# yezhen17/3DIoUMatch

Measured on AMD Instinct MI355X. Metric: scenes/sec train-step (ScanNet 40k pts, 256 proposals), higher is better.
Workload: dtype f32

## Files before the change

3dioumatch_amd/csrc/mlp_bwd_fused.hip:

```cpp
#include "common.h"
#include "mlp_operand.h"
#include "mlp_bwd_x6.h"

#ifndef MLP_LIN4_OCC
#define MLP_LIN4_OCC 1
#endif

namespace {

template <int MB, int KB, int KBD, int NB, int PMODE, int QMODE, int OCC, bool STATS, bool DGRAD = true,
          bool X6 = false>
__global__ void __launch_bounds__(256, OCC)
gemm_bwd_fused_kernel(int k_total, int r, int total_chunks, int chunks_per_cloud, int xyz,
                      OperandB opp, OperandB opq, const float *__restrict__ w,
                      float *__restrict__ dq, float *__restrict__ part,
                      float *__restrict__ stats_part) {
  constexpr int M = 32 * MB, KP = 32 * KB, TN = 32 * NB;
  constexpr int LDP = M + 1, LDQ = KP + 1;
  constexpr int TPR = TN / 16;
  constexpr int RPP = 256 / TPR;
  constexpr int PP = (M + RPP - 1) / RPP, QP = (KP + RPP - 1) / RPP;
  constexpr int WMB = MB >= 4 ? MB / 4 : 1;
  constexpr int WKB = MB >= 4 ? KB : KB * MB / 4;
  static_assert(MB >= 4 ? MB % 4 == 0 : (MB == 2 && KB % 2 == 0), "dW blocks must split over 4 waves");
// ... 285 lines not shown
#pragma unroll
            for (int n = 0; n < DN; ++n)
              accD[e][n] = __builtin_amdgcn_mfma_f32_32x32x2f32(wreg[e][g * DU + u], bp[g & 1][u][n],
                                                                accD[e][n], 0, 0, 0);
        between(g);
        __builtin_amdgcn_sched_barrier(0);
      }
      }
#pragma unroll
      for (int e = 0; e < (TF ? 0 : DK); ++e) {
        const int kbd = KBD >= 4 ? wave * DK + e : (wave >> 1);
#pragma unroll
        for (int n = 0; n < DN; ++n) {
          const int nb = KBD >= 4 ? n : (wave & 1);
          float *dst = dq + ((size_t)b * k_total + xyz + 32 * kbd + 4 * lhi) * r + col0 + nb * 32 + l31;
#pragma unroll
          for (int q = 0; q < 16; ++q)
            __builtin_nontemporal_store(accD[e][n][q], &dst[(size_t)((q & 3) + 8 * (q >> 2)) * r]);
        }
      }
    }

    auto stats_row = [&](int q) {
      const int ro = (q & 3) + 8 * (q >> 2);
      if constexpr (TF) {
#pragma unroll
        for (int e = 0; e < DK; ++e) {
          const int kbd = KBD >= 4 ? wave * DK + e : (wave >> 1);
#pragma unroll
          for (int n = 0; n < DN; ++n) {
            const int nb = KBD >= 4 ? n : (wave & 1);
            const int col = nb * 32 + 4 * lhi + ro;
            const float yv = Qc[col * LDQ + 32 * kbd + l31];
            const float g = __fmaf_rn(yv, trc[e].x, trc[e].y) > 0.f ? accD[e][n][q] : 0.f;
            st1[e][0] += g;
            st2[e][0] = __fmaf_rn(g, (yv - trc[e].z) * trc[e].w, st2[e][0]);
            const float4 xc = X4s[cur][col];
            gx[e][0] = __fmaf_rn(g, xc.x, gx[e][0]);
            gx[e][1] = __fmaf_rn(g, xc.y, gx[e][1]);
            gx[e][2] = __fmaf_rn(g, xc.z, gx[e][2]);
            gx[e][3] = __fmaf_rn(g, xc.w, gx[e][3]);
          }
        }
        return;
      }
#pragma unroll
      for (int e = 0; e < DK; ++e) {
        const int kbd = KBD >= 4 ? wave * DK + e : (wave >> 1);
        const float4 rc = Rc[32 * kbd + 4 * lhi + ro];
#pragma unroll
        for (int n = 0; n < DN; ++n) {
          const int nb = KBD >= 4 ? n : (wave & 1);
          const float yv = Qc[(nb * 32 + l31) * LDQ + 32 * kbd + 4 * lhi + ro];
          const float g = __fmaf_rn(yv, rc.x, rc.y) > 0.f ? accD[e][n][q] : 0.f;
          st1[e][STATS ? q : 0] += g;
          st2[e][STATS ? q : 0] = __fmaf_rn(g, (yv - rc.z) * rc.w, st2[e][STATS ? q : 0]);
        }
      }
    };
    if constexpr (X6) {
      float qraw[8];
      auto qfrag = [&](int g, int j) {
        const int kb = MB >= 4 ? j : (wave / MB) + (4 / MB) * j;
#pragma unroll
        for (int jj = 0; jj < 8; ++jj) {
          const float raw = Qc[(16 * g + 8 * lhi + jj) * LDQ + kb * 32 + l31];
          qraw[jj] = RAWQ ? fmaxf(__fmaf_rn(raw, fsc[j], fsh[j]), 0.f) : raw;
        }
      };
#pragma unroll
      for (int g = 0; g < WG; ++g) {
        Split3 sp[WMB];
#pragma unroll
        for (int i = 0; i < WMB; ++i) {
          const int mb = MB >= 4 ? wave + 4 * i : wave % MB;
          float praw[8];
#pragma unroll
          for (int jj = 0; jj < 8; ++jj) praw[jj] = Pc[(16 * g + 8 * lhi + jj) * LDP + mb * 32 + l31];
          sp[i] = split3(praw);
        }
        qfrag(g, 0);
#pragma unroll
        for (int j = 0; j < WKB; ++j) {
          const Split3 sq = split3(qraw);
          if (j + 1 < WKB) qfrag(g, j + 1);
#pragma unroll
          for (int i = 0; i < WMB; ++i) mfma_x6(accW[i][j], sp[i], sq);
        }
        between(DG + g);
        if (STATS) {
#pragma unroll
          for (int q = g * 16 / WG; q < (g + 1) * 16 / WG; ++q) stats_row(q);
        }
      }
    } else {
      float ap[2][WU][WMB], bq[2][WU][WKB];
      auto frag = [&](int g, float (&a)[WU][WMB], float (&bb)[WU][WKB]) {
#pragma unroll
        for (int u = 0; u < WU; ++u) {
          const int n = 2 * (g * WU + u) + lhi;
#pragma unroll
          for (int i = 0; i < WMB; ++i) {
            const int mb = MB >= 4 ? wave + 4 * i : wave % MB;
            a[u][i] = Pc[n * LDP + mb * 32 + l31];
          }
#pragma unroll
          for (int j = 0; j < WKB; ++j) {
            const int kb = MB >= 4 ? j : (wave / MB) + (4 / MB) * j;
            const float raw = Qc[n * LDQ + kb * 32 + l31];
            bb[u][j] = RAWQ ? fmaxf(__fmaf_rn(raw, fsc[j], fsh[j]), 0.f) : raw;
          }
        }
      };
      frag(0, ap[0], bq[0]);
#pragma unroll
      for (int g = 0; g < WG; ++g) {
        if (g + 1 < WG) frag(g + 1, ap[(g + 1) & 1], bq[(g + 1) & 1]);
        __builtin_amdgcn_sched_barrier(0);
#pragma unroll
        for (int u = 0; u < WU; ++u)
#pragma unroll
          for (int i = 0; i < WMB; ++i)
#pragma unroll
            for (int j = 0; j < WKB; ++j)
              accW[i][j] = __builtin_amdgcn_mfma_f32_32x32x2f32(ap[g & 1][u][i], bq[g & 1][u][j],
                                                                accW[i][j], 0, 0, 0);
        between(DG + g);
        if (STATS) {
#pragma unroll
          for (int q = g * 16 / WG; q < (g + 1) * 16 / WG; ++q) stats_row(q);
        }
        __builtin_amdgcn_sched_barrier(0);
      }
    }

    if (DGRAD && NB == 1 && xyz) {
      const int n = tid & 31, g8 = tid >> 5;
      float s0 = 0.f, s1 = 0.f, s2 = 0.f;
#pragma unroll 4
      for (int mm = g8 * (M / 8); mm < (g8 + 1) * (M / 8); ++mm) {
        const float pv = Pc[n * LDP + mm];
        s0 = __fmaf_rn(pv, Wx[mm], s0);
        s1 = __fmaf_rn(pv, Wx[M + mm], s1);
        s2 = __fmaf_rn(pv, Wx[2 * M + mm], s2);
      }
      red[(g8 * 3 + 0) * 32 + n] = s0;
      red[(g8 * 3 + 1) * 32 + n] = s1;
      red[(g8 * 3 + 2) * 32 + n] = s2;
      __syncthreads();
      if (tid < 96) {
        const int kx = tid >> 5;
        float t = 0.f;
#pragma unroll
        for (int g = 0; g < 8; ++g) t += red[(g * 3 + kx) * 32 + n];
        dq[((size_t)b * k_total + kx) * r + col0 + n] = t;
      }
    }
    __syncthreads();
  }

  if constexpr (TF) {
    constexpr int PPW = KBD >= 4 ? 1 : 2;
    const int parts = (int)gridDim.x * PPW;
    const int pidx = (int)blockIdx.x * PPW + (KBD >= 4 ? 0 : (wave & 1));
#pragma unroll
    for (int e = 0; e < DK; ++e) {
      const int row = 32 * (KBD >= 4 ? wave * DK + e : (wave >> 1)) + l31;
      float a1 = st1[e][0], a2 = st2[e][0];
      a1 += __shfl_xor(a1, 32, kWave);
      a2 += __shfl_xor(a2, 32, kWave);
      float g4[4];
#pragma unroll
      for (int k = 0; k < 4; ++k) g4[k] = gx[e][k] + __shfl_xor(gx[e][k], 32, kWave);
      if (lhi == 0) {
        if (stats_part != nullptr) {
          stats_part[((size_t)row * parts + pidx) * 2] = a1;
          stats_part[((size_t)row * parts + pidx) * 2 + 1] = a2;
        }
        *reinterpret_cast<float4 *>(dq + ((size_t)pidx * k_total + row) * 4) = make_float4(g4[0], g4[1], g4[2], g4[3]);
      }
    }
  } else if (STATS && stats_part != nullptr) {
    constexpr int PPW = KBD >= 4 ? 1 : 2;
    const int parts = (int)gridDim.x * PPW;
    const int pidx = (int)blockIdx.x * PPW + (KBD >= 4 ? 0 : (wave & 1));
#pragma unroll
    for (int e = 0; e < DK; ++e) {
      const int kbd = KBD >= 4 ? wave * DK + e : (wave >> 1);
#pragma unroll
      for (int q = 0; q < SQ; ++q) {
        float a1 = st1[e][q], a2 = st2[e][q];
#pragma unroll
        for (int off = 1; off < 32; off <<= 1) {
          a1 += __shfl_xor(a1, off, kWave);
          a2 += __shfl_xor(a2, off, kWave);
        }
        if (l31 == 0) {
          const int row = 32 * kbd + 4 * lhi + (q & 3) + 8 * (q >> 2);
          stats_part[((size_t)row * parts + pidx) * 2] = a1;
          stats_part[((size_t)row * parts + pidx) * 2 + 1] = a2;
        }
      }
    }
  }
  float *out = part + (size_t)blockIdx.x * M * k_total;
#pragma unroll
  for (int i = 0; i < WMB; ++i) {
    const int mb = MB >= 4 ? wave + 4 * i : wave % MB;
#pragma unroll
    for (int j = 0; j < WKB; ++j) {
      const int kb = MB >= 4 ? j : (wave / MB) + (4 / MB) * j;
      const int colk = kb * 32 + l31;
      if (colk >= k_total) continue;
#pragma unroll
      for (int q = 0; q < 16; ++q) {
        const int row = mb * 32 + (q & 3) + 8 * (q >> 2) + 4 * lhi;
        out[(size_t)row * k_total + colk] = accW[i][j][q];
      }
    }
  }
}

struct FusedShape { int m, k, xyz, tn, occ; };

bool fused_shape(int m, int k, FusedShape *s) {
  static const FusedShape table[] = {
      {64, 64, 0, 64, 2}, {128, 64, 0, 64, 1}, {128, 128, 0, 32, 2},
      {256, 128, 0, 32, 1}, {128, 131, 3, 32, 1}, {128, 259, 3, 32, 1},
  };
  for (const FusedShape &t : table)
    if (t.m == m && t.k == k) { *s = t; return true; }
  return false;
}

int fused_workgroups(const FusedShape &s, long long total_chunks) {
  long long g = (long long)pn2_cu_count() * s.occ;
  if (g > total_chunks / 8) g = total_chunks / 8;
  return (int)(g < 1 ? 1 : g);
}

}

#define MLP_API extern "C" __attribute__((visibility("default")))

MLP_API int mlp_gemm_backward_fused_supported(int b, int m, int k, int r, int pmode, int qmode,
                                              int ns) {
  FusedShape s;
  if (b <= 0 || r <= 0 || !fused_shape(m, k, &s)) return 0;
  if (r % s.tn != 0 || (long long)b * (r / s.tn) < 64) return 0;
  if (pmode != OP_DY && pmode != OP_POOLDY) return 0;
  if (pmode == OP_POOLDY && (ns <= 0 || ns % 16 != 0 || r % ns != 0 || (ns % s.tn != 0 && s.tn % ns != 0)))
    return 0;
  if (qmode == OP_LIN4) return m == 64 && k == 64 && pmode == OP_DY;
  const bool first = s.xyz != 0;
  if (first != (qmode == OP_DIRECT)) return 0;
  if (qmode != OP_DIRECT && qmode != OP_BNRELU) return 0;
  const bool pooled_only = (m == 128 && k == 64) || (m == 256 && k == 128);
  const bool either = m == 128 && k == 128;
  if (!either && pooled_only != (pmode == OP_POOLDY)) return 0;
  return 1;
}

MLP_API int mlp_gemm_backward_fused_stats_parts(int b, int m, int k, int r) {
  FusedShape s;
  const int gx = mlp_bwd_x6_workgroups(b, m, k, r, pn2_cu_count());
  if (gx > 0) return gx;
  if (!fused_shape(m, k, &s) || k != 64 || r % s.tn != 0) return 0;
  return fused_workgroups(s, (long long)b * (r / s.tn)) * 2;
}

MLP_API size_t mlp_gemm_backward_fused_workspace_floats(int b, int m, int k, int r) {
  FusedShape s;
  if (!fused_shape(m, k, &s) || r % s.tn != 0) return 0;
  const long long g0 = fused_workgroups(s, (long long)b * (r / s.tn));
  const long long g1 = mlp_bwd_x6_workgroups(b, m, k, r, pn2_cu_count());
  return (size_t)(g0 > g1 ? g0 : g1) * m * k;
}

MLP_API int mlp_gemm_backward_fused(int b, int m, int k, int r, const float *w, const MlpOperand *dy,
                                    const MlpOperand *x, float *dq, float *dw, float *workspace,
                                    float *stats_part, void *stream_) {
  if (b <= 0 || m <= 0 || k <= 0 || r <= 0) return 0;
  OperandB P, Q;
  int orc = operand_from_abi(dy, op_bit(OP_DY) | op_bit(OP_POOLDY), r, &P);
  if (!orc) orc = operand_from_abi(x, op_bit(OP_DIRECT) | op_bit(OP_BNRELU) | op_bit(OP_LIN4), r, &Q);
  if (orc) return orc;
  const int pmode = dy->mode, qmode = x->mode;
  if (qmode != OP_DIRECT && (!Q.mean || !Q.invstd)) return (int)hipErrorInvalidValue;
  if (!mlp_gemm_backward_fused_supported(b, m, k, r, pmode, qmode, P.ns)) return (int)hipErrorInvalidValue;
  FusedShape s;
  fused_shape(m, k, &s);
  if (dq == nullptr && !(m == 128 && k == 259)) return (int)hipErrorInvalidValue;
  hipStream_t stream = (hipStream_t)stream_;
  const int cpc = r / s.tn;
  const int total = b * cpc;
  const int g = fused_workgroups(s, total);
  {
    int gx = 0;
    const int rcx = mlp_bwd_x6_try(b, m, k, r, pmode, qmode, P, Q, w, dq, workspace,
                                   qmode == OP_BNRELU ? stats_part : nullptr, pn2_cu_count(), &gx, stream);
    if (rcx > 0) return rcx;
    if (rcx == 0) return mlp_reduce_weight_partials(m * k, gx, workspace, dw, stream);
  }
  if (k != 64) stats_part = nullptr;
#define FUSED_X(MB, KB, KBD, NB, PM, QM, OCC, ST, X6)                                           \
  hipLaunchKernelGGL((gemm_bwd_fused_kernel<MB, KB, KBD, NB, PM, QM, OCC, ST, true, X6>), dim3(g), \
                     dim3(256), 0, stream, k, r, total, cpc, s.xyz, P, Q, w, dq, workspace,     \
                     stats_part)
#define FUSED(MB, KB, KBD, NB, PM, QM, OCC, ST) FUSED_X(MB, KB, KBD, NB, PM, QM, OCC, ST, true)
#define FUSED_F32(MB, KB, KBD, NB, PM, QM, OCC, ST) FUSED_X(MB, KB, KBD, NB, PM, QM, OCC, ST, false)
  if (m == 64 && k == 64 && qmode == OP_LIN4) FUSED(2, 2, 2, 2, OP_DY, OP_LIN4, MLP_LIN4_OCC, true);
  else if (m == 64 && k == 64) FUSED(2, 2, 2, 2, OP_DY, OP_BNRELU, 2, true);
  else if (m == 128 && k == 64) FUSED(4, 2, 2, 2, OP_POOLDY, OP_BNRELU, 1, true);
  else if (m == 256 && k == 128) FUSED(8, 4, 4, 1, OP_POOLDY, OP_BNRELU, 1, false);
  else if (m == 128 && k == 131) FUSED(4, 5, 4, 1, OP_DY, OP_DIRECT, 1, false);
  else if (dq != nullptr) FUSED_F32(4, 9, 8, 1, OP_DY, OP_DIRECT, 1, false);
  else
    hipLaunchKernelGGL((gemm_bwd_fused_kernel<4, 9, 8, 1, OP_DY, OP_DIRECT, 1, false, false, true>), dim3(g),
                       dim3(256), 0, stream, k, r, total, cpc, s.xyz, P, Q, w, dq, workspace, stats_part);
#undef FUSED_F32
#undef FUSED
#undef FUSED_X
  int rc = pn2_launch_status();
  if (rc) return rc;
  return mlp_reduce_weight_partials(m * k, g, workspace, dw, stream);
}
```

3dioumatch_amd/csrc/mlp_bwd_x6.h:

```cpp
#pragma once
#include "common.h"
#include "mlp_operand.h"
#include <type_traits>

namespace {

#if defined(BWDX6_ABL) && BWDX6_ABL == 2
#define mfma_x6(ACC, A, B) do { (ACC)[0] += __builtin_bit_cast(float, (int)(A).hi[0] + (int)(B).hi[0] + (int)(A).mid[1] + (int)(B).mid[1] + (int)(A).lo[2] + (int)(B).lo[2]); } while (0)
#endif

#ifndef BWDX6_DGRAD_SLICES_STATS
#define BWDX6_DGRAD_SLICES_STATS 0xC0u
#endif
#ifndef BWDX6_DGRAD_SLICES_PLAIN
#define BWDX6_DGRAD_SLICES_PLAIN 0xF0u
#endif

constexpr int x6_popcount(unsigned v) { return v == 0 ? 0 : (int)(v & 1u) + x6_popcount(v >> 1); }

template <int MB, int KB, int KBD, int PMODE, int QMODE, bool STATS, bool DGRAD>
__device__ __forceinline__ void gemm_bwd_x6_role(int k_total, int r, int total_chunks,
                                                 int chunks_per_cloud, int xyz, const OperandB &P,
                                                 const OperandB &Q, const float *__restrict__ w,
                                                 float *__restrict__ dq, float *__restrict__ part,
// ... 64 lines not shown
      }
    }
  }

  f32x16 accW[WMB][WKB];
  if (!DGRAD) {
#pragma unroll
    for (int i = 0; i < WMB; ++i)
#pragma unroll
      for (int j = 0; j < WKB; ++j)
#pragma unroll
        for (int q = 0; q < 16; ++q) accW[i][j][q] = 0.f;
  }

  const int per = (total_chunks + (int)gridDim.x - 1) / (int)gridDim.x;
  const int c_lo = (int)blockIdx.x * per;
  const int c_hi = c_lo + per < total_chunks ? c_lo + per : total_chunks;

  float4 px[PS], pd[PS], qx[QS];
  int pwin[PS];
  float pdp[PS];
#pragma unroll
  for (int p = 0; p < PS; ++p) {
    pwin[p] = -1; pdp[p] = 0.f;
    px[p] = make_float4(0.f, 0.f, 0.f, 0.f); pd[p] = px[p];
  }
#pragma unroll
  for (int q = 0; q < QS; ++q) qx[q] = make_float4(0.f, 0.f, 0.f, 0.f);

  struct ChunkAt { size_t p, q, grp; int s0; };
  auto chunk_at = [&](int c) {
    const int b = c / chunks_per_cloud;
    const int col0 = (c - b * chunks_per_cloud) * TN;
    ChunkAt at;
    at.p = (size_t)b * M * r + col0;
    at.q = (size_t)b * k_total * r + col0;
    at.grp = 0; at.s0 = 0;
    if (PMODE == OP_POOLDY) {
      const int g0 = col0 / P.ns;
      at.grp = (size_t)b * M * P.groups + g0;
      at.s0 = col0 - g0 * P.ns;
    }
    return at;
  };
  auto fetch_slice = [&](int sl, const ChunkAt &at) {
    if (sl < PS) {
      const int p = sl;
      px[p] = *reinterpret_cast<const float4 *>(P.x + at.p + p_lane[p]);
      if (PMODE == OP_DY) {
        pd[p] = *reinterpret_cast<const float4 *>(P.dz + at.p + p_lane[p]);
      } else if (PMODE == OP_POOLDY) {
        const size_t gi = at.grp + (size_t)(seg_row + p * 32) * P.groups + lane_g;
        pwin[p] = P.argmax[gi] - (at.s0 + lane_s);
        pdp[p] = P.dz[gi];
      }
    } else {
      const int q = sl - PS;
      qx[q] = *reinterpret_cast<const float4 *>(Q.x + at.q + q_lane[q]);
    }
  };
  auto stage_slice = [&](int sl, int buf) {
    char *base = lds + (size_t)buf * BUF;
    if (sl < PS) {
      const int p = sl;
      const float xv[4] = {px[p].x, px[p].y, px[p].z, px[p].w};
      const float dv[4] = {pd[p].x, pd[p].y, pd[p].z, pd[p].w};
      float v[4];
#pragma unroll
      for (int e = 0; e < 4; ++e) {
        const float dz = PMODE == OP_POOLDY ? (e == pwin[p] ? pdp[p] : 0.f) : dv[e];
        v[e] = transform<PMODE>(xv[e], dz, pc[p]);
      }
      store_split4<RP>(base, PIMG, seg_row + p * 32, seg_c, v);
    } else {
      const int q = sl - PS;
      const float xv[4] = {qx[q].x, qx[q].y, qx[q].z, qx[q].w};
      float v[4];
#pragma unroll
      for (int e = 0; e < 4; ++e) v[e] = q_ok[q] ? transform<QMODE>(xv[e], 0.f, qc[q]) : 0.f;
      store_split4<RP>(base + 3 * PIMG, QIMG, seg_row + q * 32, seg_c, v);
      if (STATS)
        *reinterpret_cast<float4 *>(base + 3 * (PIMG + QIMG) + (size_t)(seg_row + q * 32) * RAWP + seg_c * 4) =
            qx[q];
    }
  };

  auto clampc = [&](int c) { return c < c_hi ? c : c_hi - 1; };
  if (NOWN > 0 && c_lo < c_hi) {
    const ChunkAt first = chunk_at(c_lo), second = chunk_at(clampc(c_lo + 1));
#pragma unroll
    for (int sl = 0; sl < NS; ++sl)
      if (X6_MINE(sl)) fetch_slice(sl, first);
#pragma unroll
    for (int sl = 0; sl < NS; ++sl) {
      if (!X6_MINE(sl)) continue;
      stage_slice(sl, 0);
      fetch_slice(sl, second);
    }
  }
  __syncthreads();

  const int tr_off = (8 * lhi + ((lane & 15) >> 2)) * RP + (16 * ((lane >> 4) & 1) + 4 * (lane & 3)) * 2;
  const int rw_off = l31 * RP + 8 * lhi * 2;

  auto chunk = [&](int c, int cur) {
    const char *Pc = lds + (size_t)cur * BUF, *Qc = Pc + 3 * PIMG;
    const ChunkAt ahead = chunk_at(clampc(c + 2));
    auto between = [&](int g) {
#if !defined(BWDX6_ABL) || BWDX6_ABL != 1
      int own = 0;
#pragma unroll
      for (int sl = 0; sl < NS; ++sl) {
        if (!X6_MINE(sl)) continue;
        if (own >= g * NOWN / NG && own < (g + 1) * NOWN / NG) {
#if !defined(BWDX6_ABL) || BWDX6_ABL != 7
          stage_slice(sl, cur ^ 1);
#else
          if (sl < PS) asm volatile("" :: "v"(px[sl].x), "v"(px[sl].w), "v"(pd[sl].x), "v"(pd[sl].w), "v"(pdp[sl]), "v"(pwin[sl]));
          else asm volatile("" :: "v"(qx[sl - PS].x), "v"(qx[sl - PS].w));
#endif
#if !defined(BWDX6_ABL) || BWDX6_ABL != 6
          fetch_slice(sl, ahead);
#endif
        }
        ++own;
      }
#endif
    };

    if (DGRAD) {
      const int b = c / chunks_per_cloud;
      const int col0 = (c - b * chunks_per_cloud) * TN;
      f32x16 accD[DK];
#pragma unroll
      for (int e = 0; e < DK; ++e)
#pragma unroll
        for (int q = 0; q < 16; ++q) accD[e][q] = 0.f;
      bf16x4 pf[2][3][2];
      auto frag = [&](int s, bf16x4 (&dst)[3][2]) {
#pragma unroll
        for (int t = 0; t < 3; ++t) {
          const char *p0 = Pc + (size_t)t * PIMG + (size_t)(16 * s) * RP + tr_off;
          dst[t][0] = lds_read_tr(p0);
          dst[t][1] = lds_read_tr(p0 + 4 * RP);
        }
      };
#if defined(BWDX6_ABL) && BWDX6_ABL == 3
#pragma unroll
      for (int s = 0; s < DG; ++s) between(s);
#else
      frag(0, pf[0]);
#pragma unroll
      for (int s = 0; s < DG; ++s) {
        if (s + 1 < DG) frag(s + 1, pf[(s + 1) & 1]);
        Split3 sb;
        sb.hi = __builtin_shufflevector(pf[s & 1][0][0], pf[s & 1][0][1], 0, 1, 2, 3, 4, 5, 6, 7);
        sb.mid = __builtin_shufflevector(pf[s & 1][1][0], pf[s & 1][1][1], 0, 1, 2, 3, 4, 5, 6, 7);
        sb.lo = __builtin_shufflevector(pf[s & 1][2][0], pf[s & 1][2][1], 0, 1, 2, 3, 4, 5, 6, 7);
#pragma unroll
        for (int e = 0; e < DK; ++e) mfma_x6(accD[e], wsp[e][s], sb);
        between(s);
      }
#endif
#if !defined(BWDX6_ABL) || (BWDX6_ABL != 5 && BWDX6_ABL != 3)
#pragma unroll
      for (int e = 0; e < DK; ++e) {
        const int kbd = wave * DK + e;
        float *dst = dq + ((size_t)b * k_total + xyz + 32 * kbd + 4 * lhi) * r + col0 + l31;
#pragma unroll
        for (int q = 0; q < 16; ++q) {
#if defined(BWDX6_PLAIN_STORES)
          dst[(size_t)((q & 3) + 8 * (q >> 2)) * r] = accD[e][q];
#else
          __builtin_nontemporal_store(accD[e][q], &dst[(size_t)((q & 3) + 8 * (q >> 2)) * r]);
#endif
        }
      }
#endif
      if (STATS) {
        const float4 *rc = reinterpret_cast<const float4 *>(lds + RCOFF);
        const char *raw = Pc + 3 * (PIMG + QIMG);
#pragma unroll
        for (int q = 0; q < 16; ++q) {
          const int ro = (q & 3) + 8 * (q >> 2);
#pragma unroll
          for (int e = 0; e < DK; ++e) {
            const int row = 32 * (wave * DK + e) + 4 * lhi + ro;
            const float4 c4 = rc[row];
            const float yv = *reinterpret_cast<const float *>(raw + (size_t)row * RAWP + l31 * 4);
            const float g = __fmaf_rn(yv, c4.x, c4.y) > 0.f ? accD[e][q] : 0.f;
            st1[e][q] += g;
            st2[e][q] = __fmaf_rn(g, (yv - c4.z) * c4.w, st2[e][q]);
          }
        }
      }
    } else {
      Split3 sp[WMB], sq[2];
      auto pfrag = [&](int s) {
#pragma unroll
        for (int i = 0; i < WMB; ++i) {
          const char *p0 = Pc + (size_t)((wave + 4 * i) * 32) * RP + rw_off + 16 * s * 2;
          sp[i].hi = *reinterpret_cast<const bf16x8 *>(p0);
          sp[i].mid = *reinterpret_cast<const bf16x8 *>(p0 + PIMG);
          sp[i].lo = *reinterpret_cast<const bf16x8 *>(p0 + 2 * PIMG);
        }
      };
      auto qfrag = [&](int u, Split3 &dst) {
        const int s = u / WKB, j = u % WKB;
        const char *q0 = Qc + (size_t)(j * 32) * RP + rw_off + 16 * s * 2;
        dst.hi = *reinterpret_cast<const bf16x8 *>(q0);
        dst.mid = *reinterpret_cast<const bf16x8 *>(q0 + QIMG);
        dst.lo = *reinterpret_cast<const bf16x8 *>(q0 + 2 * QIMG);
      };
#if defined(BWDX6_ABL) && BWDX6_ABL == 4
#pragma unroll
      for (int u = 0; u < WG * WKB; ++u) between(u);
#else
      pfrag(0);
      qfrag(0, sq[0]);
#pragma unroll
      for (int u = 0; u < WG * WKB; ++u) {
        const int s = u / WKB, j = u % WKB;
        if (u + 1 < WG * WKB) qfrag(u + 1, sq[(u + 1) & 1]);
#pragma unroll
        for (int i = 0; i < WMB; ++i) mfma_x6(accW[i][j], sp[i], sq[u & 1]);
        if (j == WKB - 1 && s + 1 < WG) pfrag(s + 1);
        between(u);
      }
#endif
    }
    __syncthreads();
  };
  for (int c = c_lo; c < c_hi; c += 2) {
    chunk(c, 0);
    if (c + 1 < c_hi) chunk(c + 1, 1);
  }

  if (DGRAD) {
    if (STATS && stats_part != nullptr) {
      const int parts = (int)gridDim.x;
      float2 *park = reinterpret_cast<float2 *>(lds) + (size_t)wave * (32 * DK) * 33;
#pragma unroll
      for (int e = 0; e < DK; ++e)
#pragma unroll
        for (int q = 0; q < (STATS ? 16 : 1); ++q) {
          const int lrow = 32 * e + 4 * lhi + (q & 3) + 8 * (q >> 2);
          park[lrow * 33 + l31] = make_float2(st1[e][q], st2[e][q]);
        }
      for (int t = lane; t < 32 * DK; t += kWave) {
        float a1 = 0.f, a2 = 0.f;
        for (int c2 = 0; c2 < 32; ++c2) { const float2 v = park[t * 33 + c2]; a1 += v.x; a2 += v.y; }
        const int row = 32 * wave * DK + t;
        stats_part[((size_t)row * parts + blockIdx.x) * 2] = a1;
        stats_part[((size_t)row * parts + blockIdx.x) * 2 + 1] = a2;
      }
    }
  } else {
    float *out = part + (size_t)blockIdx.x * M * k_total;
#pragma unroll
    for (int i = 0; i < WMB; ++i) {
      const int mb = wave + 4 * i;
#pragma unroll
      for (int j = 0; j < WKB; ++j) {
        const int colk = j * 32 + l31;
        if (colk >= k_total) continue;
#pragma unroll
        for (int q = 0; q < 16; ++q) {
          const int row = mb * 32 + (q & 3) + 8 * (q >> 2) + 4 * lhi;
          out[(size_t)row * k_total + colk] = accW[i][j][q];
        }
      }
    }
  }
#undef X6_MINE
}

template <int MB, int KB, int KBD, int PMODE, int QMODE, bool STATS>
__global__ void __launch_bounds__(512, 1)
gemm_bwd_x6_kernel(int k_total, int r, int total_chunks, int chunks_per_cloud, int xyz,
                   OperandB opp, OperandB opq, const float *__restrict__ w,
                   float *__restrict__ dq, float *__restrict__ part,
                   float *__restrict__ stats_part) {
  extern __shared__ __attribute__((aligned(16))) char lds[];
  const int wave = __builtin_amdgcn_readfirstlane((int)threadIdx.x >> 6);
  if (STATS) {
    constexpr int KP = 32 * KB;
    constexpr int RCOFF = 2 * (3 * (32 * MB + KP) * 80 + KP * 144);
    float4 *rc = reinterpret_cast<float4 *>(lds + RCOFF);
    for (int t = threadIdx.x; t < KP; t += 512)
      rc[t] = t < k_total ? make_float4(opq.scale[t], opq.shift[t], opq.mean[t], opq.invstd[t])
                          : make_float4(0.f, 0.f, 0.f, 0.f);
  }
  if (wave < 4) {
    gemm_bwd_x6_role<MB, KB, KBD, PMODE, QMODE, STATS, true>(
        k_total, r, total_chunks, chunks_per_cloud, xyz, opp, opq, w, dq, part, stats_part, lds,
        (int)threadIdx.x, wave);
  } else {
    gemm_bwd_x6_role<MB, KB, KBD, PMODE, QMODE, STATS, false>(
        k_total, r, total_chunks, chunks_per_cloud, xyz, opp, opq, w, dq, part, stats_part, lds,
        (int)threadIdx.x - 256, wave - 4);
  }
}

}

static int mlp_bwd_x6_workgroups(int b, int m, int k, int r, int cus) {
  if (!(m == 128 && k == 128) || r % 32 != 0 || b <= 0) return 0;
  const long long total = (long long)b * (r / 32);
  long long g = cus;
  if (g > total / 8) g = total / 8;
  return (int)(g < 1 ? 1 : g);
}

static int mlp_bwd_x6_try(int b, int m, int k, int r, int pmode, int qmode, const OperandB &P,
                          const OperandB &Q, const float *w, float *dq, float *part,
                          float *stats_part, int cus, int *workgroups, hipStream_t stream) {
  const int g = mlp_bwd_x6_workgroups(b, m, k, r, cus);
  if (g == 0 || qmode != OP_BNRELU || dq == nullptr) return -1;
  const int total_chunks = b * (r / 32), chunks_per_cloud = r / 32;
  *workgroups = g;
  constexpr int RP = 80;
#define BWDX6(MB, KB, KBD, PM, QM, ST)                                                              \
  do {                                                                                              \
    const size_t lds_bytes = 2 * (3 * (size_t)(m + k) * RP + (ST ? (size_t)k * 144 : 0)) +         \
                             (ST ? (size_t)k * 16 : 0);                                             \
    auto kern = gemm_bwd_x6_kernel<MB, KB, KBD, PM, QM, ST>;                                        \
    pn2_allow_dynamic_lds(reinterpret_cast<const void *>(kern), lds_bytes);                         \
    hipLaunchKernelGGL(kern, dim3(g), dim3(512), lds_bytes, stream, k, r, total_chunks,             \
                       chunks_per_cloud, 0, P, Q, w, dq, part, stats_part);                         \
  } while (0)
  const bool st = stats_part != nullptr;
  if (pmode == OP_DY && st) BWDX6(4, 4, 4, OP_DY, OP_BNRELU, true);
  else if (pmode == OP_DY) BWDX6(4, 4, 4, OP_DY, OP_BNRELU, false);
  else if (pmode == OP_POOLDY && st) BWDX6(4, 4, 4, OP_POOLDY, OP_BNRELU, true);
  else if (pmode == OP_POOLDY) BWDX6(4, 4, 4, OP_POOLDY, OP_BNRELU, false);
  else return -1;
#undef BWDX6
  return pn2_launch_status();
}
```

3dioumatch_amd/csrc/mlp_frag.h:

```cpp
#pragma once
#include "common.h"

namespace {

typedef float f32x16 __attribute__((ext_vector_type(16)));

typedef short bf16x8 __attribute__((ext_vector_type(8)));
typedef short bf16x4 __attribute__((ext_vector_type(4)));
struct Split3 { bf16x8 hi, mid, lo; };

__device__ __forceinline__ unsigned pack_hi16(float a, float b) {
  return __builtin_amdgcn_perm(__builtin_bit_cast(unsigned, b), __builtin_bit_cast(unsigned, a), 0x07060302u);
}

__device__ __forceinline__ void split_top(float x, float &top, float &rest) {
  top = __builtin_bit_cast(float, __builtin_bit_cast(unsigned, x) & 0xffff0000u);
  rest = x - top;
}

__device__ __forceinline__ void split_terms(float x, float &h, float &m, float &l) {
  float r1;
  split_top(x, h, r1);
  split_top(r1, m, l);
}

__device__ __forceinline__ Split3 split3(const float4 &u, const float4 &v) {
  const float x[8] = {u.x, u.y, u.z, u.w, v.x, v.y, v.z, v.w};
  float h[8], m[8], l[8];
#pragma unroll
  for (int e = 0; e < 8; ++e) split_terms(x[e], h[e], m[e], l[e]);
  typedef unsigned u32x4v __attribute__((ext_vector_type(4)));
  u32x4v ph, pm, pl;
#pragma unroll
  for (int e = 0; e < 4; ++e) {
    ph[e] = pack_hi16(h[2 * e], h[2 * e + 1]);
    pm[e] = pack_hi16(m[2 * e], m[2 * e + 1]);
    pl[e] = pack_hi16(l[2 * e], l[2 * e + 1]);
  }
  Split3 o;
  o.hi = __builtin_bit_cast(bf16x8, ph);
  o.mid = __builtin_bit_cast(bf16x8, pm);
  o.lo = __builtin_bit_cast(bf16x8, pl);
  return o;
}

__device__ __forceinline__ Split3 split3(const float (&x)[8]) {
  return split3(make_float4(x[0], x[1], x[2], x[3]), make_float4(x[4], x[5], x[6], x[7]));
}

template <int RP>
__device__ __forceinline__ void store_terms4(char *img, size_t term_bytes, int row, int c0, const float (&h)[4],
                                             const float (&m)[4], const float (&l)[4]) {
  char *dst = img + (size_t)row * RP + c0 * 2;
  *reinterpret_cast<uint2 *>(dst) = make_uint2(pack_hi16(h[0], h[1]), pack_hi16(h[2], h[3]));
  *reinterpret_cast<uint2 *>(dst + term_bytes) = make_uint2(pack_hi16(m[0], m[1]), pack_hi16(m[2], m[3]));
  *reinterpret_cast<uint2 *>(dst + 2 * term_bytes) = make_uint2(pack_hi16(l[0], l[1]), pack_hi16(l[2], l[3]));
}

template <int RP>
__device__ __forceinline__ void store_split4(char *img, size_t term_bytes, int row, int c0, const float (&v)[4]) {
  float h[4], m[4], l[4];
#pragma unroll
  for (int e = 0; e < 4; ++e) split_terms(v[e], h[e], m[e], l[e]);
  store_terms4<RP>(img, term_bytes, row, c0, h, m, l);
}

__device__ __forceinline__ void mfma_x6(f32x16 &acc, const Split3 &a, const Split3 &b) {
  acc = __builtin_amdgcn_mfma_f32_32x32x16_bf16(a.lo, b.hi, acc, 0, 0, 0);
  acc = __builtin_amdgcn_mfma_f32_32x32x16_bf16(a.hi, b.lo, acc, 0, 0, 0);
  acc = __builtin_amdgcn_mfma_f32_32x32x16_bf16(a.mid, b.mid, acc, 0, 0, 0);
  acc = __builtin_amdgcn_mfma_f32_32x32x16_bf16(a.mid, b.hi, acc, 0, 0, 0);
  acc = __builtin_amdgcn_mfma_f32_32x32x16_bf16(a.hi, b.mid, acc, 0, 0, 0);
  acc = __builtin_amdgcn_mfma_f32_32x32x16_bf16(a.hi, b.hi, acc, 0, 0, 0);
}

__device__ __forceinline__ bf16x4 lds_read_tr(const char *p) {
  return __builtin_amdgcn_ds_read_tr16_b64_v4i16(
      (__attribute__((address_space(3))) bf16x4 *)(__attribute__((address_space(3))) char *)p);
}

template <int K, int R>
__device__ __forceinline__ int img_off(int term, int t, int h, int row) {
  return (((term * (K / 16) + t) * 2 + h) * R + row) * 16;
}

__device__ __forceinline__ Split3 lds_frag(const char *p, int term_stride) {
  Split3 s;
  s.hi = *reinterpret_cast<const bf16x8 *>(p);
  s.mid = *reinterpret_cast<const bf16x8 *>(p + term_stride);
  s.lo = *reinterpret_cast<const bf16x8 *>(p + 2 * term_stride);
  return s;
}

__device__ __forceinline__ void store_frag(char *dst, int term_stride, const Split3 &s) {
  *reinterpret_cast<bf16x8 *>(dst) = s.hi;
  *reinterpret_cast<bf16x8 *>(dst + term_stride) = s.mid;
  *reinterpret_cast<bf16x8 *>(dst + 2 * term_stride) = s.lo;
}

template <int NB, bool TFORM, bool FIRST = false>
__device__ __forceinline__ void mfma6(f32x16 (&acc)[NB], const Split3 &s, const Split3 (&w)[NB]) {
  const f32x16 zero = {0.f, 0.f, 0.f, 0.f, 0.f, 0.f, 0.f, 0.f, 0.f, 0.f, 0.f, 0.f, 0.f, 0.f, 0.f, 0.f};
#define FRAG_STEP(WT, ST, C0)                                                                      \
  _Pragma("unroll") for (int i = 0; i < NB; ++i)                                                  \
    acc[i] = TFORM ? __builtin_amdgcn_mfma_f32_32x32x16_bf16(s.ST, w[i].WT, (C0) ? zero : acc[i], 0, 0, 0) \
                   : __builtin_amdgcn_mfma_f32_32x32x16_bf16(w[i].WT, s.ST, (C0) ? zero : acc[i], 0, 0, 0)
  FRAG_STEP(lo, hi, FIRST);
  FRAG_STEP(hi, lo, false);
  FRAG_STEP(mid, mid, false);
  FRAG_STEP(mid, hi, false);
  FRAG_STEP(hi, mid, false);
  FRAG_STEP(hi, hi, false);
#undef FRAG_STEP
}

constexpr int kLin4K = 64;
constexpr int kLin4ImgA = 3 * (kLin4K / 16) * 2 * 64 * 16;
constexpr int kLin4ImgB = 3 * (kLin4K / 16) * 2 * 128 * 16;
constexpr int kLin4TabW = kLin4ImgA + kLin4ImgB;
constexpr int kLin4TabC = kLin4TabW + 64 * 16;
constexpr int kLin4TabBytes = 64 * 16 + 64 * 8;
constexpr int kLin4ImgBytes = kLin4TabW + kLin4TabBytes;

}
```

Before: 1413.

## Add bf16x3-split MFMA backward kernel for pooled 256x128 MLP layer

Adds a dedicated backward kernel for the m=256,k=128 pooled-dY over BatchNorm+ReLU layer. It splits fp32 operands into three bf16 terms and runs six MFMA products each, with double-buffered swizzled LDS images and register-prefetch pipelining. Weight fragments are held in registers, pinned to accumulator registers, and dgrad is written with nontemporal stores. This replaces the generic fp32 fused kernel for this shape, trading some precision emulation and heavy register/LDS pressure for matrix-core throughput.

Result: no change. 1414, median of 3 (+0.1%).

```diff
diff --git a/3dioumatch_amd/csrc/mlp_bwd_fused.hip b/3dioumatch_amd/csrc/mlp_bwd_fused.hip
--- a/3dioumatch_amd/csrc/mlp_bwd_fused.hip
+++ b/3dioumatch_amd/csrc/mlp_bwd_fused.hip
@@ -611,6 +611,13 @@
     if (rcx > 0) return rcx;
     if (rcx == 0) return mlp_reduce_weight_partials(m * k, gx, workspace, dw, stream);
   }
+  {
+    int gp = 0;
+    const int rcp = mlp_bwd_x6_pool_try(b, m, k, r, pmode, qmode, P, Q, w, dq, workspace, pn2_cu_count(),
+                                        &gp, stream);
+    if (rcp > 0) return rcp;
+    if (rcp == 0) return mlp_reduce_weight_partials(m * k, gp, workspace, dw, stream);
+  }
   if (k != 64) stats_part = nullptr;
 #define FUSED_X(MB, KB, KBD, NB, PM, QM, OCC, ST, X6)                                           \
   hipLaunchKernelGGL((gemm_bwd_fused_kernel<MB, KB, KBD, NB, PM, QM, OCC, ST, true, X6>), dim3(g), \
@@ -621,8 +628,8 @@
   if (m == 64 && k == 64 && qmode == OP_LIN4) FUSED(2, 2, 2, 2, OP_DY, OP_LIN4, MLP_LIN4_OCC, true);
   else if (m == 64 && k == 64) FUSED(2, 2, 2, 2, OP_DY, OP_BNRELU, 2, true);
   else if (m == 128 && k == 64) FUSED(4, 2, 2, 2, OP_POOLDY, OP_BNRELU, 1, true);
-  else if (m == 256 && k == 128) FUSED(8, 4, 4, 1, OP_POOLDY, OP_BNRELU, 1, false);
   else if (m == 128 && k == 131) FUSED(4, 5, 4, 1, OP_DY, OP_DIRECT, 1, false);
+  else if (!(m == 128 && k == 259)) return (int)hipErrorInvalidValue;
   else if (dq != nullptr) FUSED_F32(4, 9, 8, 1, OP_DY, OP_DIRECT, 1, false);
   else
     hipLaunchKernelGGL((gemm_bwd_fused_kernel<4, 9, 8, 1, OP_DY, OP_DIRECT, 1, false, false, true>), dim3(g),
diff --git a/3dioumatch_amd/csrc/mlp_bwd_x6.h b/3dioumatch_amd/csrc/mlp_bwd_x6.h
--- a/3dioumatch_amd/csrc/mlp_bwd_x6.h
+++ b/3dioumatch_amd/csrc/mlp_bwd_x6.h
@@ -390,6 +390,268 @@
   }
 }
 
+constexpr int kX6PoolPitch = 64;
+__host__ __device__ constexpr int x6_pool_off(int row, int col) {
+  return row * kX6PoolPitch + ((((col >> 3) ^ (row >> 2)) & 3) << 4) + (col & 7) * 2;
+}
+
+#ifndef BWDX6_POOL_WACC
+#define BWDX6_POOL_WACC 8
+#endif
+#define X6_IN_ACC(S) asm volatile("" : "+a"((S).hi), "+a"((S).mid), "+a"((S).lo))
+template <int MB, int KB, int PMODE, int QMODE>
+__global__ void __launch_bounds__(256, 1)
+gemm_bwd_x6_pool_kernel(int r, int total_chunks, int chunks_per_cloud, OperandB P, OperandB Q,
+                        const float *__restrict__ w, float *__restrict__ dq, float *__restrict__ part) {
+  constexpr int M = 32 * MB, K = 32 * KB, TN = 32;
+  constexpr int RP = kX6PoolPitch;
+  constexpr int PIMG = M * RP, QIMG = K * RP;
+  constexpr int BUF = 3 * (PIMG + QIMG);
+  constexpr int TABP = 2 * BUF;
+  constexpr int TABPP = TABP + M * 16;
+  constexpr int TABQ = TABPP + M * 4;
+  constexpr int TABOUT = TABQ + K * 8;
+  static_assert(TABOUT + 16 <= 160 * 1024, "two buffers of images and the tables must fit the LDS");
+  static_assert(PMODE == OP_POOLDY && QMODE == OP_BNRELU, "the pooled last layer over a BatchNorm+ReLU layer");
+  static_assert(MB % 4 == 0 && KB % 4 == 0, "blocks split over four waves");
+  constexpr int WMB = MB / 4, WKB = KB;
+  constexpr int DK = KB / 4;
+  constexpr int DG = M / 16, WG = TN / 16;
+  constexpr int PS = M / 32, QS = K / 32, NS = PS + QS;
+  constexpr int NG = DG + 2 * WG * WKB;
+  constexpr int WACC = BWDX6_POOL_WACC;
+  extern __shared__ __attribute__((aligned(16))) char lds[];
+
+  const int tid = threadIdx.x, lane = tid & 63;
+  const int wave = __builtin_amdgcn_readfirstlane(tid >> 6);
+  const int l31 = lane & 31, lhi = lane >> 5;
+  const int seg_row = tid >> 3, seg_c = (tid & 7) * 4;
+
+  for (int t = tid; t < M; t += 256) {
+    const RowCoef c = load_row_coef<PMODE>(P, t, true);
+    reinterpret_cast<float4 *>(lds + TABP)[t] = make_float4(c.sc, c.sh, c.a, c.q);
+    reinterpret_cast<float *>(lds + TABPP)[t] = c.p;
+  }
+  if (tid == 0) *reinterpret_cast<float **>(lds + TABOUT) = part + (size_t)blockIdx.x * M * K;
+  for (int t = tid; t < K; t += 256) {
+    const RowCoef c = load_row_coef<QMODE>(Q, t, true);
+    reinterpret_cast<float2 *>(lds + TABQ)[t] = make_float2(c.sc, c.sh);
+  }
+
+  const unsigned x_boff = (unsigned)(seg_row * r + seg_c) * 4u;
+  const unsigned g_boff = (unsigned)(seg_row * P.groups + seg_c / P.ns) * 4u;
+  const int lane_s = seg_c % P.ns;
+  const int st_off = x6_pool_off(seg_row, seg_c);
+
+  Split3 wsp[DK][DG];
+#pragma unroll
+  for (int e = 0; e < DK; ++e) {
+    const float *wc = w + 32 * (wave * DK + e) + l31;
+#pragma unroll
+    for (int s = 0; s < DG; ++s) {
+      float w8[8];
+#pragma unroll
+      for (int j = 0; j < 8; ++j) w8[j] = wc[(size_t)(16 * s + 8 * lhi + j) * K];
+      wsp[e][s] = split3(w8);
+      if (s < WACC) X6_IN_ACC(wsp[e][s]);
+    }
+  }
+
+  f32x16 accW[WMB][WKB];
+#pragma unroll
+  for (int i = 0; i < WMB; ++i)
+#pragma unroll
+    for (int j = 0; j < WKB; ++j)
+#pragma unroll
+      for (int q = 0; q < 16; ++q) accW[i][j][q] = 0.f;
+
+  const int per = (total_chunks + (int)gridDim.x - 1) / (int)gridDim.x;
+  const int c_lo = (int)blockIdx.x * per;
+  const int c_hi = c_lo + per < total_chunks ? c_lo + per : total_chunks;
+
+  float4 px[PS], qx[QS];
+  int pwin[PS];
+  float pdp[PS];
+#pragma unroll
+  for (int p = 0; p < PS; ++p) { pwin[p] = -1; pdp[p] = 0.f; px[p] = make_float4(0.f, 0.f, 0.f, 0.f); }
+#pragma unroll
+  for (int q = 0; q < QS; ++q) qx[q] = make_float4(0.f, 0.f, 0.f, 0.f);
+
+  struct ChunkAt { size_t p, q, grp; int s0; };
+  auto chunk_at = [&](int c) {
+    const int b = c / chunks_per_cloud;
+    const int col0 = (c - b * chunks_per_cloud) * TN;
+    const int g0 = col0 / P.ns;
+    ChunkAt at;
+    at.p = (size_t)b * M * r + col0;
+    at.q = (size_t)b * K * r + col0;
+    at.grp = (size_t)b * M * P.groups + g0;
+    at.s0 = col0 - g0 * P.ns;
+    return at;
+  };
+  struct Strides { unsigned x, g; };
+  auto strides = [&]() {
+    Strides st = {(unsigned)r * 4u, (unsigned)P.groups * 4u};
+    asm volatile("" : "+s"(st.x), "+s"(st.g));
+    return st;
+  };
+  auto at_bytes = [](const void *base, unsigned boff) { return reinterpret_cast<const char *>(base) + boff; };
+  auto fetch_slice = [&](int sl, const ChunkAt &at, const Strides &st) {
+    if (sl < PS) {
+      const int p = sl;
+      px[p] = *reinterpret_cast<const float4 *>(at_bytes(P.x + at.p, p * 32 * st.x + x_boff));
+      pwin[p] = *reinterpret_cast<const int *>(at_bytes(P.argmax + at.grp, p * 32 * st.g + g_boff)) - (at.s0 + lane_s);
+      pdp[p] = *reinterpret_cast<const float *>(at_bytes(P.dz + at.grp, p * 32 * st.g + g_boff));
+    } else {
+      const int q = sl - PS;
+      qx[q] = *reinterpret_cast<const float4 *>(at_bytes(Q.x + at.q, q * 32 * st.x + x_boff));
+    }
+  };
+  auto stage_slice = [&](int sl, int buf) {
+    char *base = lds + (size_t)buf * BUF;
+    if (sl < PS) {
+      const int p = sl;
+      const float4 c4 = reinterpret_cast<const float4 *>(lds + TABP)[seg_row + p * 32];
+      const RowCoef pc = {c4.x, c4.y, c4.z, c4.w, reinterpret_cast<const float *>(lds + TABPP)[seg_row + p * 32]};
+      const float xv[4] = {px[p].x, px[p].y, px[p].z, px[p].w};
+      float v[4];
+#pragma unroll
+      for (int e = 0; e < 4; ++e) v[e] = transform<PMODE>(xv[e], e == pwin[p] ? pdp[p] : 0.f, pc);
+      store_split4_at(base + p * 32 * RP + st_off, PIMG, v);
+    } else {
+      const int q = sl - PS;
+      const float2 c2 = reinterpret_cast<const float2 *>(lds + TABQ)[seg_row + q * 32];
+      const RowCoef qc = {c2.x, c2.y, 0.f, 0.f, 0.f};
+      const float xv[4] = {qx[q].x, qx[q].y, qx[q].z, qx[q].w};
+      float v[4];
+#pragma unroll
+      for (int e = 0; e < 4; ++e) v[e] = transform<QMODE>(xv[e], 0.f, qc);
+      store_split4_at(base + 3 * PIMG + q * 32 * RP + st_off, QIMG, v);
+    }
+  };
+
+  __syncthreads();
+  auto clampc = [&](int c) { return c < c_hi ? c : c_hi - 1; };
+  if (c_lo < c_hi) {
+    const ChunkAt first = chunk_at(c_lo), second = chunk_at(clampc(c_lo + 1));
+    const Strides st = strides();
+#pragma unroll
+    for (int sl = 0; sl < NS; ++sl) fetch_slice(sl, first, st);
+#pragma unroll
+    for (int sl = 0; sl < NS; ++sl) {
+      stage_slice(sl, 0);
+      fetch_slice(sl, second, st);
+    }
+  }
+  __syncthreads();
+
+  int tr_off[2];
+#pragma unroll
+  for (int h = 0; h < 2; ++h)
+    tr_off[h] = x6_pool_off(8 * lhi + 4 * h + ((lane & 15) >> 2), 16 * ((lane >> 4) & 1) + 4 * (lane & 3));
+  int rw_off[WG];
+#pragma unroll
+  for (int s = 0; s < WG; ++s) rw_off[s] = x6_pool_off(l31, 16 * s + 8 * lhi);
+  const unsigned dq_boff = (unsigned)(4 * lhi * r + l31) * 4u;
+
+  auto chunk = [&](int c, int cur) {
+    const char *Pc = lds + (size_t)cur * BUF, *Qc = Pc + 3 * PIMG;
+    const ChunkAt ahead = chunk_at(clampc(c + 2));
+    const Strides st = strides();
+    auto between = [&](int g) {
+#pragma unroll
+      for (int sl = g * NS / NG; sl < (g + 1) * NS / NG; ++sl) {
+        stage_slice(sl, cur ^ 1);
+        fetch_slice(sl, ahead, st);
+      }
+    };
+    const int b = c / chunks_per_cloud;
+    const int col0 = (c - b * chunks_per_cloud) * TN;
+
+    {
+      f32x16 accD[DK];
+#pragma unroll
+      for (int e = 0; e < DK; ++e)
+#pragma unroll
+        for (int q = 0; q < 16; ++q) accD[e][q] = 0.f;
+      bf16x4 pf[3][2];
+      auto frag = [&](int s, bf16x4 (&dst)[3][2]) {
+#pragma unroll
+        for (int t = 0; t < 3; ++t) {
+          const char *p0 = Pc + (size_t)t * PIMG + (size_t)(16 * s) * RP;
+          dst[t][0] = lds_read_tr(p0 + tr_off[0]);
+          dst[t][1] = lds_read_tr(p0 + tr_off[1]);
+        }
+      };
+      frag(0, pf);
+#pragma unroll
+      for (int s = 0; s < DG; ++s) {
+        Split3 sb;
+        sb.hi = __builtin_shufflevector(pf[0][0], pf[0][1], 0, 1, 2, 3, 4, 5, 6, 7);
+        sb.mid = __builtin_shufflevector(pf[1][0], pf[1][1], 0, 1, 2, 3, 4, 5, 6, 7);
+        sb.lo = __builtin_shufflevector(pf[2][0], pf[2][1], 0, 1, 2, 3, 4, 5, 6, 7);
+#pragma unroll
+        for (int e = 0; e < DK; ++e) mfma_x6(accD[e], wsp[e][s], sb);
+        if (s + 1 < DG) frag(s + 1, pf);
+        between(s);
+      }
+#pragma unroll
+      for (int e = 0; e < DK; ++e) {
+        const float *dst0 = dq + ((size_t)b * K + 32 * (wave * DK + e)) * r + col0;
+#pragma unroll
+        for (int q = 0; q < 16; ++q) {
+          float *dst = reinterpret_cast<float *>(const_cast<char *>(
+              at_bytes(dst0, ((q & 3) + 8 * (q >> 2)) * st.x + dq_boff)));
+          __builtin_nontemporal_store(accD[e][q], dst);
+        }
+      }
+    }
+    {
+      Split3 sp[WMB], sq;
+      auto pfrag = [&](int s) {
+#pragma unroll
+        for (int i = 0; i < WMB; ++i)
+          sp[i] = lds_frag(Pc + (size_t)((wave + 4 * i) * 32) * RP + rw_off[s], PIMG);
+      };
+      auto qfrag = [&](int u, Split3 &dst) {
+        dst = lds_frag(Qc + (size_t)((u % WKB) * 32) * RP + rw_off[u / WKB], QIMG);
+      };
+      pfrag(0);
+      qfrag(0, sq);
+#pragma unroll
+      for (int u = 0; u < WG * WKB; ++u) {
+        const int s = u / WKB, j = u % WKB;
+#pragma unroll
+        for (int i = 0; i < WMB; ++i) mfma_x6(accW[i][j], sp[i], sq);
+        if (u + 1 < WG * WKB) qfrag(u + 1, sq);
+        if (j == WKB - 1 && s + 1 < WG) pfrag(s + 1);
+        between(DG + 2 * u);
+        between(DG + 2 * u + 1);
+      }
+    }
+    __syncthreads();
+  };
+  for (int c = c_lo; c < c_hi; c += 2) {
+    chunk(c, 0);
+    if (c + 1 < c_hi) chunk(c + 1, 1);
+  }
+
+  float *out = *reinterpret_cast<float *const *>(lds + TABOUT);
+#pragma unroll
+  for (int i = 0; i < WMB; ++i) {
+#pragma unroll
+    for (int j = 0; j < WKB; ++j) {
+#pragma unroll
+      for (int q = 0; q < 16; ++q) {
+        const int row = (wave + 4 * i) * 32 + (q & 3) + 8 * (q >> 2) + 4 * lhi;
+        out[(size_t)row * K + j * 32 + l31] = accW[i][j][q];
+      }
+    }
+  }
+}
+
+#undef X6_IN_ACC
+
 }
 
 static int mlp_bwd_x6_workgroups(int b, int m, int k, int r, int cus) {
@@ -426,3 +688,26 @@
 #undef BWDX6
   return pn2_launch_status();
 }
+
+static int mlp_bwd_x6_pool_workgroups(int b, int m, int k, int r, int cus) {
+  if (!(m == 256 && k == 128) || r % 32 != 0 || b <= 0) return 0;
+  const long long total = (long long)b * (r / 32);
+  long long g = cus;
+  if (g > total / 8) g = total / 8;
+  return (int)(g < 1 ? 1 : g);
+}
+
+static int mlp_bwd_x6_pool_try(int b, int m, int k, int r, int pmode, int qmode, const OperandB &P,
+                               const OperandB &Q, const float *w, float *dq, float *part, int cus,
+                               int *workgroups, hipStream_t stream) {
+  const int g = mlp_bwd_x6_pool_workgroups(b, m, k, r, cus);
+  if (g == 0 || pmode != OP_POOLDY || qmode != OP_BNRELU || dq == nullptr) return -1;
+  if ((long long)r * 32 * 4 >= (1ll << 32) || (long long)P.groups * 32 * 4 >= (1ll << 32))
+    return (int)hipErrorInvalidValue;
+  *workgroups = g;
+  const size_t lds_bytes = 2 * 3 * (size_t)(m + k) * kX6PoolPitch + (size_t)m * 20 + (size_t)k * 8 + 16;
+  auto kern = gemm_bwd_x6_pool_kernel<8, 4, OP_POOLDY, OP_BNRELU>;
+  pn2_allow_dynamic_lds(reinterpret_cast<const void *>(kern), lds_bytes);
+  hipLaunchKernelGGL(kern, dim3(g), dim3(256), lds_bytes, stream, r, b * (r / 32), r / 32, P, Q, w, dq, part);
+  return pn2_launch_status();
+}
diff --git a/3dioumatch_amd/csrc/mlp_frag.h b/3dioumatch_amd/csrc/mlp_frag.h
--- a/3dioumatch_amd/csrc/mlp_frag.h
+++ b/3dioumatch_amd/csrc/mlp_frag.h
@@ -65,6 +65,13 @@
   store_terms4<RP>(img, term_bytes, row, c0, h, m, l);
 }
 
+__device__ __forceinline__ void store_split4_at(char *dst, size_t term_bytes, const float (&v)[4]) {
+  float h[4], m[4], l[4];
+#pragma unroll
+  for (int e = 0; e < 4; ++e) split_terms(v[e], h[e], m[e], l[e]);
+  store_terms4<0>(dst, term_bytes, 0, 0, h, m, l);
+}
+
 __device__ __forceinline__ void mfma_x6(f32x16 &acc, const Split3 &a, const Split3 &b) {
   acc = __builtin_amdgcn_mfma_f32_32x32x16_bf16(a.lo, b.hi, acc, 0, 0, 0);
   acc = __builtin_amdgcn_mfma_f32_32x32x16_bf16(a.hi, b.lo, acc, 0, 0, 0);
```
